# cscott/compressjs

Measured on NVIDIA H100. Metric: bzip2_-9_encode_MBps, higher is better.
Workload: dtype u8

## Files before the change

### compressjs_b200/csrc/bwt_msd.cu

```cuda
#include <cstdlib>
#include <type_traits>
#include "ctx.h"
#include "tma.cuh"
#include "bwt_msd.h"

__global__ void __launch_bounds__(256)
k_msd_prep(const u32* __restrict__ hist, u32* __restrict__ bstart, u32* __restrict__ cursor, u8* __restrict__ lut, MsdBlk* __restrict__ blk,
           uint4* __restrict__ work, u32* ctl) {
  __shared__ u32 ws[9];
  __shared__ u32 s_base;
  const u32 b = blockIdx.x, d = threadIdx.x;
  const u32 h = hist[b * 256 + d];
  u32 tot;
  const u32 ex = block_excl_add<256, u32>(h, ws, &tot);
  bstart[b * 256 + d] = ex;
  cursor[b * 256 + d] = ex;
  const u32 r = block_excl_add<256, u32>(h ? 1u : 0u, ws, &tot);
  lut[b * 256 + d] = (u8)r;
  if (h > MB_CAP) atomicOr(&ctl[2], 1u);
  if (d == 0) {
    const u64 a = tot, a4 = a * a * a * a;
    MsdBlk m;
    m.a = (u32)a;
    m.a2 = (u32)(a * a);
    m.S = a4 >= (1ull << 32) ? (1ull << 32) : (a4 ? 0xffffffffffffffffull / a4 : 0ull);
    blk[b] = m;
    s_base = atomicAdd(&ctl[3], (u32)a);
  }
  __syncthreads();
  if (h) work[s_base + r] = make_uint4(b * 256 + d, ex, h, 0u);
}

struct MsdScatterSmem {
  __align__(16) u8 raw[16 + MSD_TILE + 16];
  __align__(16) u8 rk[MSD_TILE + 16];
  u32 key[MSD_TILE];
  u32 low[MSD_TILE];
  u32 cnt[256];
  int gdst[256];
  u8 lut[256];
  u32 ws[9];
  __align__(8) u64 bar;
};

__device__ __forceinline__ u32 lut4(const u8* lut, u32 w) {
  return (u32)lut[w & 0xff] | ((u32)lut[(w >> 8) & 0xff] << 8) | ((u32)lut[(w >> 16) & 0xff] << 16) | ((u32)lut[w >> 24] << 24);
}

template <int CTAS>
__global__ void __launch_bounds__(MSD_THREADS, CTAS)
k_msd_scatter(const u8* __restrict__ T, const u32* __restrict__ seg_n, u32 tps, const u8* __restrict__ lut, const MsdBlk* __restrict__ blk,
              u32* __restrict__ cursor, u64* __restrict__ rec_out, const u32* __restrict__ ctl) {
  extern __shared__ __align__(16) unsigned char smem_raw[];
  MsdScatterSmem& s = *reinterpret_cast<MsdScatterSmem*>(smem_raw);
  if (ctl[2]) return;
  const u32 b = blockIdx.x / tps, lt = blockIdx.x - b * tps;
  const u32 n = seg_n[b];
  const u32 start = lt * MSD_TILE;
  if (start >= n) return;
  const u32 count = min((u32)MSD_TILE, n - start);
  const u8* Tb = T + ((size_t)b << SEG_SHIFT);
  const u32 tid = threadIdx.x;
  if (tid == 0) {
    mbar_init(&s.bar, 1); mbar_fence_init();
    mbar_expect_tx(&s.bar, MSD_TILE);
    bulk_g2s(s.raw + 16, Tb + start, MSD_TILE, &s.bar);
  }
  const MsdBlk mb = blk[b];
  const u8 lutv = lut[b * 256 + tid];
  u8 edge = 0;
  if (tid == 32) edge = start ? Tb[start - 1] : Tb[n - 1];
  if (tid < 4) edge = Tb[(start + count + tid) % n];
  s.lut[tid] = lutv;
  s.cnt[tid] = 0;
  __syncthreads();
  mbar_wait(&s.bar, 0);
  if (tid == 32) s.raw[15] = edge;
  if (tid < 4) s.raw[16 + count + tid] = edge;
  __syncthreads();
  const u32 a = mb.a, a2 = mb.a2, S_lo = (u32)mb.S, S_hi = (u32)(mb.S >> 32);
  auto body = [&](auto full_c) {
  constexpr bool full = decltype(full_c)::value;
  const uint4 rv = *reinterpret_cast<const uint4*>(s.raw + 16 + tid * 16);
  const u32 rw[4] = {rv.x, rv.y, rv.z, rv.w};
  u32 slot[MSD_ITEMS / 2];
  {
    uint4 kv;
    kv.x = lut4(s.lut, rv.x); kv.y = lut4(s.lut, rv.y); kv.z = lut4(s.lut, rv.z); kv.w = lut4(s.lut, rv.w);
    *reinterpret_cast<uint4*>(s.rk + tid * 16) = kv;
    if (tid < 4) s.rk[count + tid] = s.lut[s.raw[16 + count + tid]];
#pragma unroll
    for (int j = 0; j < MSD_ITEMS; j++) {
      const u32 d = (rw[j >> 2] >> (8 * (j & 3))) & 0xffu;
      u32 sl = 0;
      if (full || tid * MSD_ITEMS + j < count) sl = atomicAdd(&s.cnt[d], 1u);
      if (j & 1) slot[j >> 1] |= sl << 16; else slot[j >> 1] = sl;
    }
  }
  __syncthreads();
  u32 g, ex;
  {
    const u32 c = s.cnt[tid];
    u32 tot;
    ex = block_excl_add<MSD_THREADS, u32>(c, s.ws, &tot);
    g = c ? atomicAdd(&cursor[b * 256 + tid], c) : 0u;
    s.cnt[tid] = ex;
  }
  __syncthreads();
  {
    const uint4 k0 = *reinterpret_cast<const uint4*>(s.rk + tid * 16);
    const u32 k1 = *reinterpret_cast<const u32*>(s.rk + tid * 16 + 16);
    const u32 kw[5] = {k0.x, k0.y, k0.z, k0.w, k1};
    u32 rr[20];
#pragma unroll
    for (int j = 0; j < 20; j++) rr[j] = (kw[j >> 2] >> (8 * (j & 3))) & 0xffu;
    u32 v2[19];
#pragma unroll
    for (int j = 1; j < 19; j++) v2[j] = rr[j] * a + rr[j + 1];
    u32 prev = s.raw[15 + tid * 16];
#pragma unroll
    for (int j = 0; j < MSD_ITEMS; j++) {
      const u32 d = (rw[j >> 2] >> (8 * (j & 3))) & 0xffu;
      if (full || tid * MSD_ITEMS + j < count) {
        const u32 k = v2[j + 1] * a2 + v2[j + 3];
        const u32 sl = (j & 1) ? (slot[j >> 1] >> 16) : (slot[j >> 1] & 0xffffu);
        const u32 at = s.cnt[d] + sl;
        s.key[at] = k * S_hi + __umulhi(k, S_lo);
        s.low[at] = (prev << SEG_SHIFT) | (d << 12) | (tid * MSD_ITEMS + j);
      }
      prev = d;
    }
  }
  s.gdst[tid] = (int)g - (int)ex;
  __syncthreads();
  u64* out = rec_out + ((size_t)b << SEG_SHIFT);
#pragma unroll
  for (int k = 0; k < MSD_ITEMS; k++) {
    const u32 p = k * MSD_THREADS + tid;
    if (full || p < count) {
      const u32 lw = s.low[p];
      const u32 low = (lw & 0x0ff00000u) | (start + (lw & 0xfffu));
      out[(int)p + s.gdst[(lw >> 12) & 0xffu]] = ((u64)s.key[p] << 32) | low;
    }
  }
  };
  if (count == MSD_TILE) body(std::true_type{}); else body(std::false_type{});
}

#define MB_PHASES 6
#ifdef B2_MSD_PROBE
__device__ unsigned long long g_msd_probe[MB_PHASES + 1];
#define MB_STAMP(k) do { if (tid == 0) { const long long t_ = clock64(); s.ph[k] += t_ - s.ph[MB_PHASES + 1]; s.ph[MB_PHASES + 1] = t_; } } while (0)
extern "C" __attribute__((visibility("default"))) int b2_msd_probe(unsigned long long* out) {
  unsigned long long zero[MB_PHASES + 1] = {};
  if (cudaDeviceSynchronize() != cudaSuccess || cudaMemcpyFromSymbol(out, g_msd_probe, sizeof(zero)) != cudaSuccess ||
      cudaMemcpyToSymbol(g_msd_probe, zero, sizeof(zero)) != cudaSuccess) return -1;
  return MB_PHASES;
}
#else
#define MB_STAMP(k) do { } while (0)
#endif

struct MsdBucketSmem {
  __align__(16) u64 buf[2][MB_BUF];
  __align__(16) u32 cnt[MB_CELLS / 2];
  __align__(16) u8 outb[MB_BUF + 16];
  u32 multi[MB_BUF / 2];
  __align__(8) u64 ws64[MB_THREADS / 32];
  __align__(8) u64 bar[2];
  u32 w[2], M[2], off[2], st[2];
  u32 nl[4];
#ifdef B2_MSD_PROBE
  long long ph[MB_PHASES + 2];
#endif
};

static_assert(sizeof(MsdBucketSmem) <= 227 * 1024, "bucket sort state must fit the 227 KiB of shared memory a CTA can have");


__device__ __forceinline__ u32 cell_of(u32 key) { return key >> (32 - MB_CELL_BITS); }

template <int K>
__device__ __forceinline__ void small_cell(const u64* __restrict__ buf, u32 lo, u8* __restrict__ ob, u32 base, u32 urow, u32* __restrict__ pidx,
                                           u32* __restrict__ tie_head, u32* __restrict__ tie_idx, u32* ctl) {
  u64 v[K];
#pragma unroll
  for (int i = 0; i < K; i++) v[i] = buf[lo + i];
#pragma unroll
  for (int round = 0; round < K; round++) {
#pragma unroll
    for (int i = round & 1; i + 1 < K; i += 2) {
      const u64 a = v[i], b = v[i + 1];
      const bool sw = a > b;
      v[i] = sw ? b : a;
      v[i + 1] = sw ? a : b;
    }
  }
  bool any_tie = false;
#pragma unroll
  for (int i = 0; i < K; i++) {
    const u32 lw = (u32)v[i];
    ob[lo + i] = (u8)(lw >> SEG_SHIFT);
    if ((lw & SEG_MASK) == 0) pidx[base >> SEG_SHIFT] = urow + lo + i;
    if (i + 1 < K) any_tie |= (u32)(v[i] >> 32) == (u32)(v[i + 1] >> 32);
  }
  if (any_tie) {
    int run0 = 0;
#pragma unroll
    for (int i = 0; i < K; i++) {
      if (i + 1 == K || (u32)(v[i + 1] >> 32) != (u32)(v[i] >> 32)) {
        const int run = i + 1 - run0;
        if (run > 1) {
          u32 t = atomicAdd(&ctl[0], (u32)run);
          const u32 head = base | (urow + lo + run0);
#pragma unroll
          for (int z = 0; z < K; z++)
            if (z >= run0 && z <= i) { tie_head[t] = head; tie_idx[t] = base | ((u32)v[z] & SEG_MASK); t++; }
        }
        run0 = i + 1;
      }
    }
  }
}

__device__ __forceinline__ void big_cell(const u64* __restrict__ cb, u32 size, u32 lo, u8* __restrict__ ob, u32 base, u32 urow,
                                         u32* __restrict__ pidx, u32* __restrict__ tie_head, u32* __restrict__ tie_idx, u32* ctl,
                                         u16* __restrict__ rank) {
  const u32 lane = threadIdx.x & 31u;
  for (u32 e0 = 0; e0 < size; e0 += 32) {
    const u32 e = e0 + lane;
    if (e < size) {
      const u64 x = cb[e];
      u32 less = 0;
      for (u32 q = 0; q < size; q++) less += cb[q] < x ? 1u : 0u;
      const u32 lw = (u32)x;
      ob[lo + less] = (u8)(lw >> SEG_SHIFT);
      if ((lw & SEG_MASK) == 0) pidx[base >> SEG_SHIFT] = urow + lo + less;
      rank[less] = (u16)e;
    }
  }
  __syncwarp();
  if (lane == 0) {
    u32 run0 = 0;
    for (u32 r = 0; r < size; r++) {
      const u32 kr = (u32)(cb[rank[r]] >> 32);
      if (r + 1 == size || (u32)(cb[rank[r + 1]] >> 32) != kr) {
        const u32 run = r + 1 - run0;
        if (run > 1) {
          u32 t = atomicAdd(&ctl[0], run);
          const u32 head = base | (urow + lo + run0);
          for (u32 z = run0; z <= r; z++) { tie_head[t] = head; tie_idx[t] = base | ((u32)cb[rank[z]] & SEG_MASK); t++; }
        }
        run0 = r + 1;
      }
    }
  }
  __syncwarp();
}

__device__ __forceinline__ u64 scan_excl_1barrier(u64 v, u64* ws, u64* total) {
  static_assert(MB_THREADS == 1024, "one lane per warp total");
  const u64 inc = warp_incl_add(v);
  const u32 w = threadIdx.x >> 5, l = threadIdx.x & 31u;
  if (l == 31) ws[w] = inc;
  __syncthreads();
  const u64 x = ws[l];
  const u64 xi = warp_incl_add(x);
  const u64 before = __shfl_sync(FULL_MASK, xi - x, (int)w);
  *total = __shfl_sync(FULL_MASK, xi, 31);
  return before + inc - v;
}

__global__ void __launch_bounds__(MB_THREADS, 1)
k_msd_bucket(const u64* __restrict__ rec, const uint4* __restrict__ work, u8* __restrict__ U, u32* __restrict__ pidx,
             u32* __restrict__ tie_head, u32* __restrict__ tie_idx, u32* ctl) {
  extern __shared__ __align__(16) unsigned char smem_raw[];
  MsdBucketSmem& s = *reinterpret_cast<MsdBucketSmem*>(smem_raw);
  if (ctl[2]) return;
  const u32 tid = threadIdx.x;
  const u32 nw = ctl[3];
  auto issue = [&](u32 i, uint4 d) {
    const u32 w = d.x, st = d.y, M = d.z, off = st & 1u;
    s.w[i] = w; s.M[i] = M; s.off[i] = off; s.st[i] = st;
    if (!M) return;
    const u32 recs = (M + off + 1u) & ~1u;
    mbar_expect_tx(&s.bar[i], recs * 8u);
    bulk_g2s(s.buf[i], rec + (((size_t)(w >> 8)) << SEG_SHIFT) + (st - off), recs * 8u, &s.bar[i]);
  };
  uint4 dnext = make_uint4(0, 0, 0, 0);
  u32 inext = blockIdx.x + gridDim.x;
  if (tid == 0) {
    mbar_init(&s.bar[0], 1); mbar_init(&s.bar[1], 1); mbar_fence_init();
    issue(0, blockIdx.x < nw ? work[blockIdx.x] : dnext);
    if (inext < nw) dnext = work[inext];
  }
  auto clear_cells = [&]() {
    const uint4 z = make_uint4(0, 0, 0, 0);
    uint4* c4 = reinterpret_cast<uint4*>(s.cnt);
#pragma unroll
    for (u32 k = 0; k < MB_CELLS / 8 / MB_THREADS; k++) c4[tid + k * MB_THREADS] = z;
  };
  clear_cells();
  __syncthreads();
#ifdef B2_MSD_PROBE
  if (tid == 0) {
    for (int k = 0; k <= MB_PHASES; k++) s.ph[k] = 0;
    s.ph[MB_PHASES + 1] = clock64();
  }
#endif
  for (u32 it = 0;; it++) {
    const u32 i = it & 1u;
    if (s.M[i] == 0) break;
    const u32 w = s.w[i];
    if (tid == 0) {
      issue(i ^ 1u, dnext);
      inext += gridDim.x;
      dnext = inext < nw ? work[inext] : make_uint4(0, 0, 0, 0);
    }
    const u32 M = s.M[i], off = s.off[i], ust = s.st[i], blockb = w >> 8;
    u64* buf = s.buf[i];
    mbar_wait(&s.bar[i], (it >> 1) & 1u);
    u64 r[MB_ITEMS];
#pragma unroll
    for (int k = 0; k < MB_ITEMS; k++) {
      const u32 p = tid + k * MB_THREADS;
      r[k] = p < M ? buf[off + p] : 0ull;
    }
    MB_STAMP(0);
#pragma unroll
    for (int k = 0; k < MB_ITEMS; k++) {
      const u32 p = tid + k * MB_THREADS;
      if (p < M) {
        const u32 c = cell_of((u32)(r[k] >> 32));
        atomicAdd(&s.cnt[c >> 1], 1u << ((c & 1u) * 16u));
      }
    }
    __syncthreads();
    MB_STAMP(1);
    u8* ob = s.outb + (ust & 15u);
    {
      uint4* c4 = reinterpret_cast<uint4*>(s.cnt) + tid * 2;
      uint4 x0 = c4[0], x1 = c4[1];
      u32 wv[8] = {x0.x, x0.y, x0.z, x0.w, x1.x, x1.y, x1.z, x1.w};
      const u32 H = 0x00010001u;
      u32 sum = 0, a2 = 0, a3 = 0, a4 = 0, a5 = 0, mm = 0;
#pragma unroll
      for (int k = 0; k < 8; k++) {
        const u32 w = wv[k];
        sum += (w & 0xffffu) + (w >> 16);
        const u32 ge2 = ((w + 0x7ffe7ffeu) >> 15) & H;
        a2 += ge2;
        a3 += ((w + 0x7ffd7ffdu) >> 15) & H;
        a4 += ((w + 0x7ffc7ffcu) >> 15) & H;
        a5 += ((w + 0x7ffb7ffbu) >> 15) & H;
        mm |= ge2 << k;
      }
      const u32 g2 = (a2 & 0xffffu) + (a2 >> 16), g3 = (a3 & 0xffffu) + (a3 >> 16), g4 = (a4 & 0xffffu) + (a4 >> 16), g5 = (a5 & 0xffffu) + (a5 >> 16);
      u64 tot;
      const u64 ex = scan_excl_1barrier((u64)sum | ((u64)(g2 - g3) << 14) | ((u64)(g3 - g4) << 27) | ((u64)(g4 - g5) << 39) | ((u64)g5 << 51),
                                        s.ws64, &tot);
      const u32 t2 = (u32)(tot >> 14) & 0x1fffu, t3 = (u32)(tot >> 27) & 0xfffu, t4 = (u32)(tot >> 39) & 0xfffu, tN = (u32)(tot >> 51);
      if (tid == 0) { s.nl[0] = t2; s.nl[1] = t3; s.nl[2] = t4; s.nl[3] = tN; }
      u32 run = (u32)ex & 0x3fffu;
#pragma unroll
      for (int k = 0; k < 8; k++) {
        const u32 w = wv[k];
        const u32 s1 = run + (w & 0xffffu);
        const u32 one = (((w + 0x7fff7fffu) >> 15) & H) & ~((w + 0x7ffe7ffeu) >> 15);
        wv[k] = (run | (s1 << 16)) | (one << 15);
        run = s1 + (w >> 16);
      }
      c4[0] = make_uint4(wv[0], wv[1], wv[2], wv[3]);
      c4[1] = make_uint4(wv[4], wv[5], wv[6], wv[7]);
      __syncwarp();
      u32 i2 = (u32)(ex >> 14) & 0x1fffu, i3 = t2 + ((u32)(ex >> 27) & 0xfffu), i4 = t2 + t3 + ((u32)(ex >> 39) & 0xfffu),
          iN = t2 + t3 + t4 + (u32)(ex >> 51);
      const u16* cst = reinterpret_cast<const u16*>(s.cnt) + tid * 16;
      while (mm) {
        const u32 b = __ffs(mm) - 1;
        mm &= mm - 1;
        const u32 c = 2 * (b & 15u) + (b >> 4);
        const u32 st = cst[c] & 0x3fffu;
        const u32 nx = c == 15 ? run : (cst[c + 1] & 0x3fffu);
        const u32 size = nx - st;
        const u32 at = size == 2 ? i2++ : (size == 3 ? i3++ : (size == 4 ? i4++ : iN++));
        s.multi[at] = st | (size << 16);
      }
    }
    __syncthreads();
    MB_STAMP(2);
#pragma unroll
    for (int k = 0; k < MB_ITEMS; k++) {
      const u32 p = tid + k * MB_THREADS;
      if (p < M) {
        const u32 c = cell_of((u32)(r[k] >> 32));
        const u32 sh = (c & 1u) * 16u;
        const u32 half = (atomicAdd(&s.cnt[c >> 1], 1u << sh) >> sh) & 0xffffu;
        const u32 pos = half & 0x7fffu;
        if (half & 0x8000u) {
          const u32 lw = (u32)r[k];
          ob[pos] = (u8)(lw >> SEG_SHIFT);
          if ((lw & SEG_MASK) == 0) pidx[blockb] = ust + pos;
        } else {
          buf[pos] = r[k];
        }
      }
    }
    __syncthreads();
    MB_STAMP(3);
    {
      const u32 n2 = s.nl[0], n3 = s.nl[1], n4 = s.nl[2], nN = s.nl[3];
      const u32 base = (blockb << SEG_SHIFT), urow = ust;
      const u32 rt = MB_THREADS - 1 - tid;
      for (u32 j = rt >> 5; j < nN; j += MB_THREADS / 32) {
        const u32 mmv = s.multi[n2 + n3 + n4 + j], lo = mmv & 0xffffu, size = mmv >> 16;
        if (size > MB_MAXCELL) { if ((tid & 31u) == 0) atomicOr(&ctl[1], 1u); continue; }
        big_cell(buf + lo, size, lo, ob, base, urow, pidx, tie_head, tie_idx, ctl, reinterpret_cast<u16*>(s.cnt) + lo);
      }
      for (u32 j = rt; j < n4; j += MB_THREADS) small_cell<4>(buf, s.multi[n2 + n3 + j] & 0xffffu, ob, base, urow, pidx, tie_head, tie_idx, ctl);
      for (u32 j = (tid + MB_THREADS / 2) & (MB_THREADS - 1); j < n3; j += MB_THREADS)
        small_cell<3>(buf, s.multi[n2 + j] & 0xffffu, ob, base, urow, pidx, tie_head, tie_idx, ctl);
      for (u32 j = tid; j < n2; j += MB_THREADS) small_cell<2>(buf, s.multi[j] & 0xffffu, ob, base, urow, pidx, tie_head, tie_idx, ctl);
    }
    __syncthreads();
    MB_STAMP(4);
    {
      const u32 first = ust & 15u, last = first + M;
      u8* Ug = U + ((size_t)blockb << SEG_SHIFT) + (ust - first);
      for (u32 c16 = tid * 16u; c16 < last; c16 += MB_THREADS * 16u) {
        if (c16 >= first && c16 + 16u <= last) {
          *reinterpret_cast<uint4*>(Ug + c16) = *reinterpret_cast<const uint4*>(s.outb + c16);
        } else {
          const u32 e = min(c16 + 16u, last);
          for (u32 x = max(c16, first); x < e; x++) Ug[x] = s.outb[x];
        }
      }
    }
    clear_cells();
    fence_async_smem();
    __syncthreads();
    MB_STAMP(5);
#ifdef B2_MSD_PROBE
    if (tid == 0) s.ph[MB_PHASES]++;
#endif
  }
#ifdef B2_MSD_PROBE
  if (tid == 0)
    for (int k = 0; k <= MB_PHASES; k++) atomicAdd(&g_msd_probe[k], (unsigned long long)s.ph[k]);
#endif
}

void bwt_msd_launch(Ctx& c, const u8* d_T, u8* d_U, const u32* d_n, u32 nblk, u32 n_max, u64 n_total, const u32* d_hist, u64* d_rec,
                    u32* d_pidx, u32* d_tie_head, u32* d_tie_idx, u32* d_ctl) {
  static int sms = 0, scatter_ctas = MSD_CTAS_PER_SM;
  if (!sms) {
    CUDA_CHECK(cudaDeviceGetAttribute(&sms, cudaDevAttrMultiProcessorCount, c.device));
    CUDA_CHECK(cudaFuncSetAttribute(k_msd_scatter<4>, cudaFuncAttributeMaxDynamicSharedMemorySize, (int)sizeof(MsdScatterSmem)));
    CUDA_CHECK(cudaFuncSetAttribute(k_msd_scatter<5>, cudaFuncAttributeMaxDynamicSharedMemorySize, (int)sizeof(MsdScatterSmem)));
    if (const char* e = getenv("B2_MSD_CTAS")) scatter_ctas = atoi(e) == 4 ? 4 : 5;
    CUDA_CHECK(cudaFuncSetAttribute(k_msd_bucket, cudaFuncAttributeMaxDynamicSharedMemorySize, (int)sizeof(MsdBucketSmem)));
  }
  DBuf<u32> bstart(c, (size_t)nblk * 256), cursor(c, (size_t)nblk * 256);
  DBuf<u8> lut(c, (size_t)nblk * 256);
  DBuf<MsdBlk> blk(c, nblk);
  DBuf<uint4> work(c, (size_t)nblk * 256);
  k_msd_prep<<<nblk, 256, 0, c.stream>>>(d_hist, bstart, cursor, lut, blk, work, d_ctl);
  KLAUNCH(c); KCHECK();
  const u32 tps = (n_max + MSD_TILE - 1) / MSD_TILE;
  {
    size_t ev = c.begin(ST_MSD_SCATTER);
    if (scatter_ctas == 4) k_msd_scatter<4><<<tps * nblk, MSD_THREADS, sizeof(MsdScatterSmem), c.stream>>>(d_T, d_n, tps, lut, blk, cursor, d_rec, d_ctl);
    else k_msd_scatter<5><<<tps * nblk, MSD_THREADS, sizeof(MsdScatterSmem), c.stream>>>(d_T, d_n, tps, lut, blk, cursor, d_rec, d_ctl);
    c.end(ev);
    KLAUNCH(c); KCHECK();
    ev = c.begin(ST_MSD_BUCKET);
    k_msd_bucket<<<(unsigned)sms, MB_THREADS, sizeof(MsdBucketSmem), c.stream>>>(d_rec, work, d_U, d_pidx, d_tie_head, d_tie_idx, d_ctl);
    c.end(ev);
    KLAUNCH(c); KCHECK();
  }
  c.stats.msd_launches++;
  c.stats.msd_scatter_bytes += n_total * 9;
  c.stats.msd_bucket_bytes += n_total * 9;
  c.stats.bwt_bytes += n_total * 18;
}
```

Measured before the change: 28000.

## Derive in-cell ranks from histogram atomics and build multi-cell lists during counting

The counting pass now keeps the return value of the per-cell shared atomic as each record's rank within its cell, packed as 10-bit fields. The scatter pass uses that rank instead of a second round of atomics. Cells with two or more and with five or more entries are appended to worklists during counting through warp-aggregated atomics, which removes the 64-bit packed multi-count scan and the per-thread cell enumeration. big_cell also skips its serial tie-run scan when a warp vote finds no equal adjacent keys. In exchange small cells of sizes 2-4 now run through one mixed loop with branches, and the ranks cost extra registers.

```diff
diff --git a/compressjs_b200/csrc/bwt_msd.cu b/compressjs_b200/csrc/bwt_msd.cu
--- a/compressjs_b200/csrc/bwt_msd.cu
+++ b/compressjs_b200/csrc/bwt_msd.cu
@@ -166,10 +166,10 @@
   __align__(16) u32 cnt[MB_CELLS / 2];
   __align__(16) u8 outb[MB_BUF + 16];
   u32 multi[MB_BUF / 2];
-  __align__(8) u64 ws64[MB_THREADS / 32];
+  u32 ws[MB_THREADS / 32];
   __align__(8) u64 bar[2];
   u32 w[2], M[2], off[2], st[2];
-  u32 nl[4];
+  u32 nq[2];
 #ifdef B2_MSD_PROBE
   long long ph[MB_PHASES + 2];
 #endif
@@ -240,6 +240,9 @@
     }
   }
   __syncwarp();
+  bool tie = false;
+  for (u32 r = lane; r + 1 < size; r += 32) tie |= (u32)(cb[rank[r]] >> 32) == (u32)(cb[rank[r + 1]] >> 32);
+  if (!__any_sync(FULL_MASK, tie)) return;
   if (lane == 0) {
     u32 run0 = 0;
     for (u32 r = 0; r < size; r++) {
@@ -258,16 +261,15 @@
   __syncwarp();
 }
 
-__device__ __forceinline__ u64 scan_excl_1barrier(u64 v, u64* ws, u64* total) {
+__device__ __forceinline__ u32 scan_excl_1barrier(u32 v, u32* ws) {
   static_assert(MB_THREADS == 1024, "one lane per warp total");
-  const u64 inc = warp_incl_add(v);
+  const u32 inc = warp_incl_add(v);
   const u32 w = threadIdx.x >> 5, l = threadIdx.x & 31u;
   if (l == 31) ws[w] = inc;
   __syncthreads();
-  const u64 x = ws[l];
-  const u64 xi = warp_incl_add(x);
-  const u64 before = __shfl_sync(FULL_MASK, xi - x, (int)w);
-  *total = __shfl_sync(FULL_MASK, xi, 31);
+  const u32 x = ws[l];
+  const u32 xi = warp_incl_add(x);
+  const u32 before = __shfl_sync(FULL_MASK, xi - x, (int)w);
   return before + inc - v;
 }
 
@@ -301,6 +303,7 @@
     for (u32 k = 0; k < MB_CELLS / 8 / MB_THREADS; k++) c4[tid + k * MB_THREADS] = z;
   };
   clear_cells();
+  if (tid == 0) { s.nq[0] = 0; s.nq[1] = 0; }
   __syncthreads();
 #ifdef B2_MSD_PROBE
   if (tid == 0) {
@@ -327,13 +330,33 @@
       r[k] = p < M ? buf[off + p] : 0ull;
     }
     MB_STAMP(0);
-#pragma unroll
-    for (int k = 0; k < MB_ITEMS; k++) {
-      const u32 p = tid + k * MB_THREADS;
-      if (p < M) {
-        const u32 c = cell_of((u32)(r[k] >> 32));
-        atomicAdd(&s.cnt[c >> 1], 1u << ((c & 1u) * 16u));
-      }
+    u32 rk[(MB_ITEMS + 2) / 3];
+    {
+      u32 m2 = 0, m5 = 0;
+#pragma unroll
+      for (int k = 0; k < MB_ITEMS; k++) {
+        const u32 p = tid + k * MB_THREADS;
+        u32 rank = 0xffffu;
+        if (p < M) {
+          const u32 c = cell_of((u32)(r[k] >> 32)), sh = (c & 1u) * 16u;
+          rank = (atomicAdd(&s.cnt[c >> 1], 1u << sh) >> sh) & 0xffffu;
+        }
+        const u32 f = (rank & 0x3ffu) << (10 * (k % 3));
+        rk[k / 3] = k % 3 ? rk[k / 3] | f : f;
+        m2 |= (rank == 1u ? 1u : 0u) << k;
+        m5 |= (rank == 4u ? 1u : 0u) << k;
+      }
+      auto append = [&](u32 m, u32 list) {
+        const u32 n = __popc(m), inc = warp_incl_add(n);
+        u32 at = 0;
+        if ((tid & 31u) == 31u && inc) at = atomicAdd(&s.nq[list], inc);
+        at = __shfl_sync(FULL_MASK, at, 31) + inc - n;
+#pragma unroll
+        for (int k = 0; k < MB_ITEMS; k++)
+          if ((m >> k) & 1u) s.multi[list ? MB_BUF / 2 - 1 - at++ : at++] = cell_of((u32)(r[k] >> 32));
+      };
+      append(m2, 0);
+      if (__any_sync(FULL_MASK, m5)) append(m5, 1);
     }
     __syncthreads();
     MB_STAMP(1);
@@ -343,25 +366,10 @@
       uint4 x0 = c4[0], x1 = c4[1];
       u32 wv[8] = {x0.x, x0.y, x0.z, x0.w, x1.x, x1.y, x1.z, x1.w};
       const u32 H = 0x00010001u;
-      u32 sum = 0, a2 = 0, a3 = 0, a4 = 0, a5 = 0, mm = 0;
-#pragma unroll
-      for (int k = 0; k < 8; k++) {
-        const u32 w = wv[k];
-        sum += (w & 0xffffu) + (w >> 16);
-        const u32 ge2 = ((w + 0x7ffe7ffeu) >> 15) & H;
-        a2 += ge2;
-        a3 += ((w + 0x7ffd7ffdu) >> 15) & H;
-        a4 += ((w + 0x7ffc7ffcu) >> 15) & H;
-        a5 += ((w + 0x7ffb7ffbu) >> 15) & H;
-        mm |= ge2 << k;
-      }
-      const u32 g2 = (a2 & 0xffffu) + (a2 >> 16), g3 = (a3 & 0xffffu) + (a3 >> 16), g4 = (a4 & 0xffffu) + (a4 >> 16), g5 = (a5 & 0xffffu) + (a5 >> 16);
-      u64 tot;
-      const u64 ex = scan_excl_1barrier((u64)sum | ((u64)(g2 - g3) << 14) | ((u64)(g3 - g4) << 27) | ((u64)(g4 - g5) << 39) | ((u64)g5 << 51),
-                                        s.ws64, &tot);
-      const u32 t2 = (u32)(tot >> 14) & 0x1fffu, t3 = (u32)(tot >> 27) & 0xfffu, t4 = (u32)(tot >> 39) & 0xfffu, tN = (u32)(tot >> 51);
-      if (tid == 0) { s.nl[0] = t2; s.nl[1] = t3; s.nl[2] = t4; s.nl[3] = tN; }
-      u32 run = (u32)ex & 0x3fffu;
+      u32 both = 0;
+#pragma unroll
+      for (int k = 0; k < 8; k++) both += wv[k];
+      u32 run = scan_excl_1barrier((both & 0xffffu) + (both >> 16), s.ws);
 #pragma unroll
       for (int k = 0; k < 8; k++) {
         const u32 w = wv[k];
@@ -372,55 +380,50 @@
       }
       c4[0] = make_uint4(wv[0], wv[1], wv[2], wv[3]);
       c4[1] = make_uint4(wv[4], wv[5], wv[6], wv[7]);
-      __syncwarp();
-      u32 i2 = (u32)(ex >> 14) & 0x1fffu, i3 = t2 + ((u32)(ex >> 27) & 0xfffu), i4 = t2 + t3 + ((u32)(ex >> 39) & 0xfffu),
-          iN = t2 + t3 + t4 + (u32)(ex >> 51);
-      const u16* cst = reinterpret_cast<const u16*>(s.cnt) + tid * 16;
-      while (mm) {
-        const u32 b = __ffs(mm) - 1;
-        mm &= mm - 1;
-        const u32 c = 2 * (b & 15u) + (b >> 4);
-        const u32 st = cst[c] & 0x3fffu;
-        const u32 nx = c == 15 ? run : (cst[c + 1] & 0x3fffu);
-        const u32 size = nx - st;
-        const u32 at = size == 2 ? i2++ : (size == 3 ? i3++ : (size == 4 ? i4++ : iN++));
-        s.multi[at] = st | (size << 16);
-      }
     }
     __syncthreads();
     MB_STAMP(2);
-#pragma unroll
-    for (int k = 0; k < MB_ITEMS; k++) {
-      const u32 p = tid + k * MB_THREADS;
-      if (p < M) {
-        const u32 c = cell_of((u32)(r[k] >> 32));
-        const u32 sh = (c & 1u) * 16u;
-        const u32 half = (atomicAdd(&s.cnt[c >> 1], 1u << sh) >> sh) & 0xffffu;
-        const u32 pos = half & 0x7fffu;
-        if (half & 0x8000u) {
-          const u32 lw = (u32)r[k];
-          ob[pos] = (u8)(lw >> SEG_SHIFT);
-          if ((lw & SEG_MASK) == 0) pidx[blockb] = ust + pos;
-        } else {
-          buf[pos] = r[k];
+    {
+      const u16* cst = reinterpret_cast<const u16*>(s.cnt);
+#pragma unroll
+      for (int k = 0; k < MB_ITEMS; k++) {
+        const u32 p = tid + k * MB_THREADS;
+        if (p < M) {
+          const u32 st = cst[cell_of((u32)(r[k] >> 32))];
+          if (st & 0x8000u) {
+            const u32 lw = (u32)r[k], pos = st & 0x7fffu;
+            ob[pos] = (u8)(lw >> SEG_SHIFT);
+            if ((lw & SEG_MASK) == 0) pidx[blockb] = ust + pos;
+          } else {
+            buf[st + ((rk[k / 3] >> (10 * (k % 3))) & 0x3ffu)] = r[k];
+          }
         }
       }
+      const u32 nS = s.nq[0], nB = s.nq[1];
+      auto rows = [&](u32 at) {
+        const u32 c = s.multi[at], lo = cst[c];
+        const u32 hi = c + 1 < MB_CELLS ? (u32)cst[c + 1] & 0x7fffu : M;
+        s.multi[at] = lo | ((hi - lo) << 16);
+      };
+      for (u32 j = tid; j < nS; j += MB_THREADS) rows(j);
+      for (u32 j = tid; j < nB; j += MB_THREADS) rows(MB_BUF / 2 - 1 - j);
     }
     __syncthreads();
     MB_STAMP(3);
     {
-      const u32 n2 = s.nl[0], n3 = s.nl[1], n4 = s.nl[2], nN = s.nl[3];
+      const u32 nS = s.nq[0], nB = s.nq[1];
       const u32 base = (blockb << SEG_SHIFT), urow = ust;
-      const u32 rt = MB_THREADS - 1 - tid;
-      for (u32 j = rt >> 5; j < nN; j += MB_THREADS / 32) {
-        const u32 mmv = s.multi[n2 + n3 + n4 + j], lo = mmv & 0xffffu, size = mmv >> 16;
+      for (u32 j = (MB_THREADS - 1 - tid) >> 5; j < nB; j += MB_THREADS / 32) {
+        const u32 mmv = s.multi[MB_BUF / 2 - 1 - j], lo = mmv & 0xffffu, size = mmv >> 16;
         if (size > MB_MAXCELL) { if ((tid & 31u) == 0) atomicOr(&ctl[1], 1u); continue; }
         big_cell(buf + lo, size, lo, ob, base, urow, pidx, tie_head, tie_idx, ctl, reinterpret_cast<u16*>(s.cnt) + lo);
       }
-      for (u32 j = rt; j < n4; j += MB_THREADS) small_cell<4>(buf, s.multi[n2 + n3 + j] & 0xffffu, ob, base, urow, pidx, tie_head, tie_idx, ctl);
-      for (u32 j = (tid + MB_THREADS / 2) & (MB_THREADS - 1); j < n3; j += MB_THREADS)
-        small_cell<3>(buf, s.multi[n2 + j] & 0xffffu, ob, base, urow, pidx, tie_head, tie_idx, ctl);
-      for (u32 j = tid; j < n2; j += MB_THREADS) small_cell<2>(buf, s.multi[j] & 0xffffu, ob, base, urow, pidx, tie_head, tie_idx, ctl);
+      for (u32 j = tid; j < nS; j += MB_THREADS) {
+        const u32 mmv = s.multi[j], lo = mmv & 0xffffu, size = mmv >> 16;
+        if (size == 2) small_cell<2>(buf, lo, ob, base, urow, pidx, tie_head, tie_idx, ctl);
+        else if (size == 3) small_cell<3>(buf, lo, ob, base, urow, pidx, tie_head, tie_idx, ctl);
+        else if (size == 4) small_cell<4>(buf, lo, ob, base, urow, pidx, tie_head, tie_idx, ctl);
+      }
     }
     __syncthreads();
     MB_STAMP(4);
@@ -437,6 +440,7 @@
       }
     }
     clear_cells();
+    if (tid == 0) { s.nq[0] = 0; s.nq[1] = 0; }
     fence_async_smem();
     __syncthreads();
     MB_STAMP(5);
```

Result: faster. 28300, median of 6 (+1.1%).

## Reuse histogram atomic slots for scatter and rebuild multi-cell queue construction

Applied to the files above, without the earlier changes.

The counting-pass atomics now keep their returned per-cell slot in registers, so the scatter pass reads the cell starts without a second round of shared-memory atomics. The cell scan is reduced to a 32-bit, one-barrier prefix sum. Multi-element cells are staged compactly and then sorted into size-class queues using warp ballots, replacing the per-thread bitmask walk. big_cell also counts equal keys and skips the serial tie-recording loop when no ties exist, which costs one extra comparison per element.

```diff
diff --git a/compressjs_b200/csrc/bwt_msd.cu b/compressjs_b200/csrc/bwt_msd.cu
--- a/compressjs_b200/csrc/bwt_msd.cu
+++ b/compressjs_b200/csrc/bwt_msd.cu
@@ -165,11 +165,13 @@
   __align__(16) u64 buf[2][MB_BUF];
   __align__(16) u32 cnt[MB_CELLS / 2];
   __align__(16) u8 outb[MB_BUF + 16];
-  u32 multi[MB_BUF / 2];
-  __align__(8) u64 ws64[MB_THREADS / 32];
+  u16 q23[MB_BUF / 2];
+  u32 q4n[MB_BUF / 4];
+  u32 ws[MB_THREADS / 32];
   __align__(8) u64 bar[2];
   u32 w[2], M[2], off[2], st[2];
-  u32 nl[4];
+  u32 nw;
+  __align__(16) u32 nl[4];
 #ifdef B2_MSD_PROBE
   long long ph[MB_PHASES + 2];
 #endif
@@ -227,12 +229,17 @@
                                          u32* __restrict__ pidx, u32* __restrict__ tie_head, u32* __restrict__ tie_idx, u32* ctl,
                                          u16* __restrict__ rank) {
   const u32 lane = threadIdx.x & 31u;
+  u32 equal = 0;
   for (u32 e0 = 0; e0 < size; e0 += 32) {
     const u32 e = e0 + lane;
     if (e < size) {
       const u64 x = cb[e];
-      u32 less = 0;
-      for (u32 q = 0; q < size; q++) less += cb[q] < x ? 1u : 0u;
+      u32 less = 0, eq = 0;
+      for (u32 q = 0; q < size; q++) {
+        less += cb[q] < x ? 1u : 0u;
+        eq += (u32)(cb[q] >> 32) == (u32)(x >> 32) ? 1u : 0u;
+      }
+      equal = max(equal, eq);
       const u32 lw = (u32)x;
       ob[lo + less] = (u8)(lw >> SEG_SHIFT);
       if ((lw & SEG_MASK) == 0) pidx[base >> SEG_SHIFT] = urow + lo + less;
@@ -240,7 +247,8 @@
     }
   }
   __syncwarp();
-  if (lane == 0) {
+  const bool tied = __any_sync(FULL_MASK, equal > 1);
+  if (tied && lane == 0) {
     u32 run0 = 0;
     for (u32 r = 0; r < size; r++) {
       const u32 kr = (u32)(cb[rank[r]] >> 32);
@@ -258,17 +266,15 @@
   __syncwarp();
 }
 
-__device__ __forceinline__ u64 scan_excl_1barrier(u64 v, u64* ws, u64* total) {
+__device__ __forceinline__ u32 scan_excl_1barrier(u32 v, u32* ws) {
   static_assert(MB_THREADS == 1024, "one lane per warp total");
-  const u64 inc = warp_incl_add(v);
+  const u32 inc = warp_incl_add(v);
   const u32 w = threadIdx.x >> 5, l = threadIdx.x & 31u;
   if (l == 31) ws[w] = inc;
   __syncthreads();
-  const u64 x = ws[l];
-  const u64 xi = warp_incl_add(x);
-  const u64 before = __shfl_sync(FULL_MASK, xi - x, (int)w);
-  *total = __shfl_sync(FULL_MASK, xi, 31);
-  return before + inc - v;
+  const u32 x = ws[l];
+  const u32 xi = warp_incl_add(x);
+  return __shfl_sync(FULL_MASK, xi - x, (int)w) + inc - v;
 }
 
 __global__ void __launch_bounds__(MB_THREADS, 1)
@@ -278,7 +284,6 @@
   MsdBucketSmem& s = *reinterpret_cast<MsdBucketSmem*>(smem_raw);
   if (ctl[2]) return;
   const u32 tid = threadIdx.x;
-  const u32 nw = ctl[3];
   auto issue = [&](u32 i, uint4 d) {
     const u32 w = d.x, st = d.y, M = d.z, off = st & 1u;
     s.w[i] = w; s.M[i] = M; s.off[i] = off; s.st[i] = st;
@@ -287,12 +292,13 @@
     mbar_expect_tx(&s.bar[i], recs * 8u);
     bulk_g2s(s.buf[i], rec + (((size_t)(w >> 8)) << SEG_SHIFT) + (st - off), recs * 8u, &s.bar[i]);
   };
+  auto entry = [&](u32 it) { const u32 e = blockIdx.x + it * gridDim.x; return e < s.nw ? work[e] : make_uint4(0, 0, 0, 0); };
   uint4 dnext = make_uint4(0, 0, 0, 0);
-  u32 inext = blockIdx.x + gridDim.x;
   if (tid == 0) {
     mbar_init(&s.bar[0], 1); mbar_init(&s.bar[1], 1); mbar_fence_init();
-    issue(0, blockIdx.x < nw ? work[blockIdx.x] : dnext);
-    if (inext < nw) dnext = work[inext];
+    s.nw = ctl[3];
+    issue(0, entry(0));
+    dnext = entry(1);
   }
   auto clear_cells = [&]() {
     const uint4 z = make_uint4(0, 0, 0, 0);
@@ -311,92 +317,96 @@
   for (u32 it = 0;; it++) {
     const u32 i = it & 1u;
     if (s.M[i] == 0) break;
-    const u32 w = s.w[i];
     if (tid == 0) {
       issue(i ^ 1u, dnext);
-      inext += gridDim.x;
-      dnext = inext < nw ? work[inext] : make_uint4(0, 0, 0, 0);
-    }
-    const u32 M = s.M[i], off = s.off[i], ust = s.st[i], blockb = w >> 8;
+      dnext = entry(it + 2);
+    }
+    const u32 M = s.M[i], off = s.off[i];
     u64* buf = s.buf[i];
     mbar_wait(&s.bar[i], (it >> 1) & 1u);
     u64 r[MB_ITEMS];
 #pragma unroll
     for (int k = 0; k < MB_ITEMS; k++) {
       const u32 p = tid + k * MB_THREADS;
-      r[k] = p < M ? buf[off + p] : 0ull;
+      r[k] = p < M ? buf[off + p] : (u64)tid << (32 + 32 - MB_CELL_BITS);
     }
     MB_STAMP(0);
+    u32 slot[MB_ITEMS / 2];
 #pragma unroll
     for (int k = 0; k < MB_ITEMS; k++) {
-      const u32 p = tid + k * MB_THREADS;
-      if (p < M) {
-        const u32 c = cell_of((u32)(r[k] >> 32));
-        atomicAdd(&s.cnt[c >> 1], 1u << ((c & 1u) * 16u));
-      }
+      const u32 c = cell_of((u32)(r[k] >> 32)), sh = (c & 1u) * 16u;
+      const u32 sl = (atomicAdd(&s.cnt[c >> 1], tid + k * MB_THREADS < M ? 1u << sh : 0u) >> sh) & 0xffffu;
+      if (k & 1) slot[k >> 1] |= sl << 16; else slot[k >> 1] = sl;
     }
     __syncthreads();
     MB_STAMP(1);
-    u8* ob = s.outb + (ust & 15u);
     {
       uint4* c4 = reinterpret_cast<uint4*>(s.cnt) + tid * 2;
-      uint4 x0 = c4[0], x1 = c4[1];
-      u32 wv[8] = {x0.x, x0.y, x0.z, x0.w, x1.x, x1.y, x1.z, x1.w};
       const u32 H = 0x00010001u;
-      u32 sum = 0, a2 = 0, a3 = 0, a4 = 0, a5 = 0, mm = 0;
-#pragma unroll
-      for (int k = 0; k < 8; k++) {
-        const u32 w = wv[k];
-        sum += (w & 0xffffu) + (w >> 16);
-        const u32 ge2 = ((w + 0x7ffe7ffeu) >> 15) & H;
-        a2 += ge2;
-        a3 += ((w + 0x7ffd7ffdu) >> 15) & H;
-        a4 += ((w + 0x7ffc7ffcu) >> 15) & H;
-        a5 += ((w + 0x7ffb7ffbu) >> 15) & H;
-        mm |= ge2 << k;
-      }
-      const u32 g2 = (a2 & 0xffffu) + (a2 >> 16), g3 = (a3 & 0xffffu) + (a3 >> 16), g4 = (a4 & 0xffffu) + (a4 >> 16), g5 = (a5 & 0xffffu) + (a5 >> 16);
-      u64 tot;
-      const u64 ex = scan_excl_1barrier((u64)sum | ((u64)(g2 - g3) << 14) | ((u64)(g3 - g4) << 27) | ((u64)(g4 - g5) << 39) | ((u64)g5 << 51),
-                                        s.ws64, &tot);
-      const u32 t2 = (u32)(tot >> 14) & 0x1fffu, t3 = (u32)(tot >> 27) & 0xfffu, t4 = (u32)(tot >> 39) & 0xfffu, tN = (u32)(tot >> 51);
-      if (tid == 0) { s.nl[0] = t2; s.nl[1] = t3; s.nl[2] = t4; s.nl[3] = tN; }
-      u32 run = (u32)ex & 0x3fffu;
-#pragma unroll
-      for (int k = 0; k < 8; k++) {
-        const u32 w = wv[k];
-        const u32 s1 = run + (w & 0xffffu);
-        const u32 one = (((w + 0x7fff7fffu) >> 15) & H) & ~((w + 0x7ffe7ffeu) >> 15);
-        wv[k] = (run | (s1 << 16)) | (one << 15);
-        run = s1 + (w >> 16);
-      }
-      c4[0] = make_uint4(wv[0], wv[1], wv[2], wv[3]);
-      c4[1] = make_uint4(wv[4], wv[5], wv[6], wv[7]);
+      const u32 sw = (tid >> 2) & 1u;
+      u32 half0, both;
+      {
+        auto tally = [&](const uint4 x) {
+          const u32 sum = x.x + x.y + x.z + x.w;
+          const u32 q = (((x.x + 0x7ffe7ffeu) >> 15) & H) + (((x.y + 0x7ffe7ffeu) >> 15) & H) +
+                        (((x.z + 0x7ffe7ffeu) >> 15) & H) + (((x.w + 0x7ffe7ffeu) >> 15) & H);
+          return (sum & 0xffffu) + (sum >> 16) + (q << 16) + (q & 0xffff0000u);
+        };
+        const u32 ta = tally(c4[sw]), tb = tally(c4[sw ^ 1u]);
+        half0 = sw ? tb : ta;
+        both = ta + tb;
+      }
+      if (tid == 0) *reinterpret_cast<uint4*>(s.nl) = make_uint4(0, 0, 0, 0);
+      const u32 ex = scan_excl_1barrier(both, s.ws);
+      u32* const stage = reinterpret_cast<u32*>(buf);
+#pragma unroll
+      for (int j = 0; j < 2; j++) {
+        const u32 h = sw ^ (u32)j;
+        const uint4 x = c4[h];
+        u32 wv[4] = {x.x, x.y, x.z, x.w};
+        u32 run = (ex & 0xffffu) + (h ? half0 & 0xffffu : 0u);
+        u32* at = stage + (ex >> 16) + (h ? half0 >> 16 : 0u);
+#pragma unroll
+        for (int k = 0; k < 4; k++) {
+          const u32 w = wv[k];
+          const u32 s1 = run + (w & 0xffffu);
+          const u32 ge2 = ((w + 0x7ffe7ffeu) >> 15) & H;
+          const u32 one = (((w + 0x7fff7fffu) >> 15) & H) & ~ge2;
+          wv[k] = (run | (s1 << 16)) | (one << 15);
+          if (ge2 & 1u) *at++ = run | (w << 16);
+          if (ge2 >> 16) *at++ = s1 | (w & 0xffff0000u);
+          run = s1 + (w >> 16);
+        }
+        c4[h] = make_uint4(wv[0], wv[1], wv[2], wv[3]);
+      }
       __syncwarp();
-      u32 i2 = (u32)(ex >> 14) & 0x1fffu, i3 = t2 + ((u32)(ex >> 27) & 0xfffu), i4 = t2 + t3 + ((u32)(ex >> 39) & 0xfffu),
-          iN = t2 + t3 + t4 + (u32)(ex >> 51);
-      const u16* cst = reinterpret_cast<const u16*>(s.cnt) + tid * 16;
-      while (mm) {
-        const u32 b = __ffs(mm) - 1;
-        mm &= mm - 1;
-        const u32 c = 2 * (b & 15u) + (b >> 4);
-        const u32 st = cst[c] & 0x3fffu;
-        const u32 nx = c == 15 ? run : (cst[c + 1] & 0x3fffu);
-        const u32 size = nx - st;
-        const u32 at = size == 2 ? i2++ : (size == 3 ? i3++ : (size == 4 ? i4++ : iN++));
-        s.multi[at] = st | (size << 16);
+      const u32 lane = tid & 31u, end = __shfl_sync(FULL_MASK, (ex + both) >> 16, 31);
+      for (u32 e0 = __shfl_sync(FULL_MASK, ex >> 16, 0); e0 < end; e0 += 32) {
+        const u32 v = e0 + lane < end ? stage[e0 + lane] : 0u, size = v >> 16;
+        const u32 cls = size ? min(size, 5u) - 2u : 0u;
+        const u32 have = __ballot_sync(FULL_MASK, size != 0), b0 = __ballot_sync(FULL_MASK, cls & 1u),
+                  b1 = __ballot_sync(FULL_MASK, cls & 2u);
+        auto lanes_of = [&](u32 k) { return have & ((k & 1u) ? b0 : ~b0) & ((k & 2u) ? b1 : ~b1); };
+        const u32 lk = lanes_of(lane);
+        u32 base = 0;
+        if (lane < 4 && lk) base = atomicAdd(&s.nl[lane], (u32)__popc(lk));
+        const u32 pos = __shfl_sync(FULL_MASK, base, (int)cls) + __popc(lanes_of(cls) & ((1u << lane) - 1u));
+        if (size) {
+          if (cls < 2) s.q23[cls ? MB_BUF / 2 - 1 - pos : pos] = (u16)v;
+          else s.q4n[cls == 2 ? pos : MB_BUF / 4 - 1 - pos] = v;
+        }
       }
     }
     __syncthreads();
     MB_STAMP(2);
+    const u16* cstart = reinterpret_cast<const u16*>(s.cnt);
+    const u32 blockb = s.w[i] >> 8, ust = s.st[i];
+    u8* ob = s.outb + (ust & 15u);
 #pragma unroll
     for (int k = 0; k < MB_ITEMS; k++) {
-      const u32 p = tid + k * MB_THREADS;
-      if (p < M) {
-        const u32 c = cell_of((u32)(r[k] >> 32));
-        const u32 sh = (c & 1u) * 16u;
-        const u32 half = (atomicAdd(&s.cnt[c >> 1], 1u << sh) >> sh) & 0xffffu;
-        const u32 pos = half & 0x7fffu;
+      const u32 half = cstart[cell_of((u32)(r[k] >> 32))];
+      if (tid + k * MB_THREADS < M) {
+        const u32 pos = (half & 0x7fffu) + ((slot[k >> 1] >> ((k & 1) * 16)) & 0xffffu);
         if (half & 0x8000u) {
           const u32 lw = (u32)r[k];
           ob[pos] = (u8)(lw >> SEG_SHIFT);
@@ -413,14 +423,14 @@
       const u32 base = (blockb << SEG_SHIFT), urow = ust;
       const u32 rt = MB_THREADS - 1 - tid;
       for (u32 j = rt >> 5; j < nN; j += MB_THREADS / 32) {
-        const u32 mmv = s.multi[n2 + n3 + n4 + j], lo = mmv & 0xffffu, size = mmv >> 16;
+        const u32 mmv = s.q4n[MB_BUF / 4 - 1 - j], lo = mmv & 0xffffu, size = mmv >> 16;
         if (size > MB_MAXCELL) { if ((tid & 31u) == 0) atomicOr(&ctl[1], 1u); continue; }
         big_cell(buf + lo, size, lo, ob, base, urow, pidx, tie_head, tie_idx, ctl, reinterpret_cast<u16*>(s.cnt) + lo);
       }
-      for (u32 j = rt; j < n4; j += MB_THREADS) small_cell<4>(buf, s.multi[n2 + n3 + j] & 0xffffu, ob, base, urow, pidx, tie_head, tie_idx, ctl);
+      for (u32 j = rt; j < n4; j += MB_THREADS) small_cell<4>(buf, s.q4n[j] & 0xffffu, ob, base, urow, pidx, tie_head, tie_idx, ctl);
       for (u32 j = (tid + MB_THREADS / 2) & (MB_THREADS - 1); j < n3; j += MB_THREADS)
-        small_cell<3>(buf, s.multi[n2 + j] & 0xffffu, ob, base, urow, pidx, tie_head, tie_idx, ctl);
-      for (u32 j = tid; j < n2; j += MB_THREADS) small_cell<2>(buf, s.multi[j] & 0xffffu, ob, base, urow, pidx, tie_head, tie_idx, ctl);
+        small_cell<3>(buf, s.q23[MB_BUF / 2 - 1 - j], ob, base, urow, pidx, tie_head, tie_idx, ctl);
+      for (u32 j = tid; j < n2; j += MB_THREADS) small_cell<2>(buf, s.q23[j], ob, base, urow, pidx, tie_head, tie_idx, ctl);
     }
     __syncthreads();
     MB_STAMP(4);
```

After: 28360 before, 28970 after (median of 6 runs). +2.2%, better.
